# YuePanEdward/MULLS

Measured on NVIDIA H100. Metric: scan-pair registrations/sec (120k-pt 64-beam), higher is better.
Workload: dtype f32 geometry / f64 accumulation

## Files before the change

### mulls_b200/csrc/kernels_iterate.cuh

```cuda
#pragma once
#include <cooperative_groups.h>

#include "device_math.cuh"
#include "device_types.cuh"
#include "kernels_ingest.cuh"

namespace mulls {

__device__ __forceinline__ bool chunk_in_run(const DeviceArrays &A) { return blockIdx.x < (unsigned)A.ctl->n_it_chunks; }
__device__ __forceinline__ int loop_buf(const DeviceArrays &A, int buf) { return buf >= 0 ? buf : (A.ctl->it & 1); }
__device__ __forceinline__ mulls_icp_trace *trace_of(const DeviceArrays &A, uint32_t pair) {
    return (A.trace && A.ctl->trace_on) ? &A.trace[pair] : nullptr;
}

template <class Body>
__device__ __forceinline__ void for_each_live_chunk(const DeviceArrays &A, int parity, int which, Body body) {
    __shared__ uint32_t s_fetch;
    LoopCtl &ctl = *A.ctl;
    const uint32_t n = ctl.n_live[parity];
    const uint32_t *list = A.live_chunks + (size_t)parity * A.live_stride;
    for (;;) {
        __syncthreads();
        if (threadIdx.x == 0) s_fetch = atomicAdd(&ctl.work[which], 1u);
        __syncthreads();
// ... 482 lines not shown
    t[19] = (-wx * py * pz);
    t[20] = wx * py * py + wy * px * px;
    t[21] = (-wx * dx);
    t[22] = (-wy * dy);
    t[23] = (-wz * dz);
    t[24] = wy * pz * dy - wz * py * dz;
    t[25] = wz * px * dz - wx * pz * dx;
    t[26] = wx * py * dx - wy * px * dy;
}

__device__ __forceinline__ float balanced_ground_weight(const PairConst &pc, const uint32_t *n_corr) {
    if (!pc.w_balance) return 1.0f;
    const int m1 = (int)(n_corr[MULLS_GROUND] + n_corr[MULLS_ROOF]);
    const int m2 = (int)n_corr[MULLS_FACADE], m3 = (int)n_corr[MULLS_PILLAR], m4 = (int)n_corr[MULLS_BEAM];
    const float num = pc.z_xy_ratio * (float)(m2 + 2 * m3 - m4);
    const double v = (double)num / (0.0001 + 2.0 * (double)m1);
    return (float)((0.01 > v) ? 0.01 : v);
}

__device__ __forceinline__ bool too_few(const PairConst &pc, const PairState &ps, const uint32_t *n_corr, float &ratio) {
    int total = 0;
    for (int c = 0; c < kNumClasses; ++c) total += (int)n_corr[c];
    const int nec = (int)(n_corr[MULLS_PILLAR] + n_corr[MULLS_BEAM] + n_corr[MULLS_FACADE]);
    ratio = (float)(1.0 * (double)nec / (double)ps.source_feature_points_count);
    return total < 40 || nec < 20 || ratio < pc.min_ratio;
}

__device__ __forceinline__ void pair_left_running(DeviceArrays &A) {
    const int left = atomicSub(A.running, 1) - 1;
    *A.h_running = left;
    __threadfence_system();
}

__device__ __noinline__ void solve_and_advance(DeviceArrays &A, uint32_t pair, const double *S, double *sm ,
                                  int buf_written) {
    const PairConst &pc = A.pc[pair];
    PairState &ps = A.ps[pair];
    const int i = ps.iter;
    ps.iters_entered = i + 1;
    for (int c = 0; c < kNumClasses; ++c) ps.n_corr_last[c] = ps.n_corr[c];
    {
        uint64_t pts = 0;
        for (int c = 0; c < kNumClasses; ++c)
            if (pc.used[c]) pts += (uint64_t)ps.n_tgt[c];
        ps.alg_bytes += 28ull * pts;
    }
    mulls_icp_trace *tr = trace_of(A, pair);
    if (tr && i < MULLS_MAX_TRACE_ITERS) {
        tr->n_iter = i + 1;
        for (int c = 0; c < kNumClasses; ++c) tr->n_corr[i][c] = ps.n_corr[c];
        for (int k = 0; k < 36; ++k) tr->atpa[i][k] = 0.0;
        for (int k = 0; k < 6; ++k) tr->atpb[i][k] = tr->x[i][k] = 0.0;
    }
    float ratio;
    const bool few = too_few(pc, ps, ps.n_corr, ratio);
    ps.confidence = ratio;
    if (few) {
        ps.code = -2;
        ps.status = kDone;
        pair_left_running(A);
        return;
    }
    {
        const double t = 1.0 * (double)ps.thre / (double)pc.thre_rate;
        ps.thre = (t > (double)pc.thre_min) ? (float)t : pc.thre_min;
    }
    double *ATPA = sm;
    double *ATPb = sm + 36;
    double *inv = sm + 42;
    double *lu = sm + 78;
    double *Tmp = sm + 114;
    double low[21];
    for (int k = 0; k < 21; ++k) low[k] = 0.0;
    for (int k = 0; k < 6; ++k) ATPb[k] = 0.0;
    const int order[6] = {MULLS_GROUND, MULLS_FACADE, MULLS_ROOF, MULLS_PILLAR, MULLS_BEAM, MULLS_VERTEX};
    for (int o = 0; o < 6; ++o) {
        const double *s = S + order[o] * kTerms;
        for (int k = 0; k < 21; ++k) low[k] += s[k];
        for (int k = 0; k < 6; ++k) ATPb[k] += s[21 + k];
    }
    {
        int k = 0;
        for (int col = 0; col < 6; ++col)
            for (int row = col; row < 6; ++row, ++k) {
                ATPA[6 * row + col] = low[k];
                ATPA[6 * col + row] = low[k];
            }
    }
    inverse6(ATPA, inv, lu);
    double x[6];
    for (int r = 0; r < 6; ++r) {
        double s = inv[6 * r] * ATPb[0];
        for (int cc = 1; cc < 6; ++cc) s = s + inv[6 * r + cc] * ATPb[cc];
        x[r] = s;
        ps.x[r] = s;
    }
    if (tr && i < MULLS_MAX_TRACE_ITERS) {
        for (int k = 0; k < 36; ++k) tr->atpa[i][k] = ATPA[k];
        for (int k = 0; k < 6; ++k) {
            tr->atpb[i][k] = ATPb[k];
            tr->x[i][k] = x[k];
        }
    }
    {
        const float sr = (float)sin(0.5 * x[3]), sp = (float)sin(0.5 * x[4]), sy = (float)sin(0.5 * x[5]);
        const float cr = (float)cos(0.5 * x[3]), cp = (float)cos(0.5 * x[4]), cy = (float)cos(0.5 * x[5]);
        double J[3][3];
        J[0][0] = 0.5 * (double)(cr * cp * cy + sr * sp * sy);
        J[0][1] = 0.5 * (double)(-sr * sp * cy - cr * cp * sy);
        J[0][2] = 0.5 * (double)(-sr * cp * sy - cr * sp * cy);
        J[1][0] = 0.5 * (double)(-sr * sp * cy + cr * cp * sy);
        J[1][1] = 0.5 * (double)(cr * cp * cy - sr * sp * sy);
        J[1][2] = 0.5 * (double)(-cr * sp * sy + sr * cp * cy);
        J[2][0] = 0.5 * (double)(-sr * cp * sy - cr * sp * cy);
        J[2][1] = 0.5 * (double)(-cr * sp * sy - sr * cp * cy);
        J[2][2] = 0.5 * (double)(cr * cp * cy + sr * sp * sy);
        double *cof = ps.cofactor;
        for (int k = 0; k < 36; ++k) cof[k] = inv[k];
        double tmp[3][3];
        for (int r = 0; r < 3; ++r)
            for (int cc = 0; cc < 3; ++cc)
                tmp[r][cc] = J[r][0] * inv[6 * 3 + 3 + cc] + J[r][1] * inv[6 * 4 + 3 + cc] + J[r][2] * inv[6 * 5 + 3 + cc];
        for (int r = 0; r < 3; ++r)
            for (int cc = 0; cc < 3; ++cc)
                cof[6 * (3 + r) + 3 + cc] = tmp[r][0] * J[cc][0] + tmp[r][1] * J[cc][1] + tmp[r][2] * J[cc][2];
        for (int r = 0; r < 3; ++r)
            for (int cc = 0; cc < 3; ++cc)
                cof[6 * r + 3 + cc] = inv[6 * r + 3] * J[cc][0] + inv[6 * r + 4] * J[cc][1] + inv[6 * r + 5] * J[cc][2];
        for (int r = 0; r < 3; ++r)
            for (int cc = 0; cc < 3; ++cc)
                cof[6 * (3 + r) + cc] = J[r][0] * inv[6 * 3 + cc] + J[r][1] * inv[6 * 4 + cc] + J[r][2] * inv[6 * 5 + cc];
    }
    double *Tt = ps.T_inc;
    construct_trans_a(x, Tt);
    const double ts_norm = sqrt(Tt[3] * Tt[3] + Tt[7] * Tt[7] + Tt[11] * Tt[11]);
    const double rs_angle = fabs(rotation_angle(Tt));
    if (ts_norm > (double)pc.max_t || rs_angle > (double)pc.max_r) {
        ps.code = -1;
        ps.status = kDone;
        pair_left_running(A);
        return;
    }
    mat4_mul(Tt, ps.T_total, Tmp);
    for (int k = 0; k < 16; ++k) ps.T_total[k] = Tmp[k];
    if (i == pc.max_iter - 1 || (i > 2 && ts_norm < (double)pc.conv_t && rs_angle < (double)pc.conv_r)) {
        ps.status = kNeedPosterior;
        ps.final_buf = buf_written;
        pair_left_running(A);
        return;
    }
    ps.iter = i + 1;
}

__device__ __forceinline__ void accumulate_body(DeviceArrays &A, int buf, uint32_t chunk) {
    const ChunkDesc cd = A.it_chunks[chunk];
    const PairConst &pc = A.pc[cd.pair];
    PairState &ps = A.ps[cd.pair];
    if (ps.status != kRunning) return;
    const int c = (int)cd.seg;
    const int ns = ps.n_src[c];
    const uint32_t local = cd.first + threadIdx.x;
    const bool valid = (int)local < ns;
    const int lane = threadIdx.x & 31, warp = threadIdx.x >> 5;
    constexpr int kWarps = kIterBlock / 32;
    __shared__ double s_terms[27 * kIterBlock];
    __shared__ uint32_t s_off[kWarps + 1];
    __shared__ uint32_t s_base;

    if ((int)cd.first >= ns) return;
    uint32_t dst_local = 0;
    uint8_t fl = 0;
    uint32_t gi = 0;
    bool kept = false, pass = false;
    struct Column {
        double *base;
        __device__ __forceinline__ double &operator[](int k) const { return base[k * kIterBlock]; }
    } t = {s_terms + threadIdx.x};
    {
        uint32_t acc = 0;
        const uint32_t first_chunk = pc.class_chunk_begin[c];
        for (uint32_t b = first_chunk + threadIdx.x; b < chunk; b += kIterBlock) acc += A.blk_kept[b];
        for (int o = 16; o > 0; o >>= 1) acc += __shfl_xor_sync(0xffffffffu, acc, o);
        if (lane == 0) s_off[warp] = acc;
        __syncthreads();
        if (threadIdx.x == 0) {
            uint32_t tt = 0;
            for (int w = 0; w < kWarps; ++w) tt += s_off[w];
            s_base = tt;
        }
        __syncthreads();
    }
    if (valid) {
        gi = pc.src_base[c] + local;
        fl = A.flags[gi];
    }
    kept = (fl & 1) != 0, pass = (fl & 2) != 0;
    const unsigned kb = __ballot_sync(0xffffffffu, kept);
    if (lane == 0) s_off[warp] = __popc(kb);
    __syncthreads();
    if (threadIdx.x == 0) {
        uint32_t run = 0;
        for (int w = 0; w < kWarps; ++w) {
            const uint32_t tt = s_off[w];
            s_off[w] = run;
            run += tt;
        }
        s_off[kWarps] = run;
    }
    __syncthreads();
    dst_local = s_base + s_off[warp] + __popc(kb & ((1u << lane) - 1u));

    float4 p = make_float4(0, 0, 0, 0);
    int j = -1;
    float d2 = 0.0f;
    const uint32_t gd = pc.src_base[c] + dst_local;
    if (kept) {
        p = advanced_pos(ps, A.src_pos[buf][gi]);
        j = A.nn_idx[gi];
        d2 = A.nn_d2[gi];
        if (j >= 0) A.claim[pc.tgt_base[c] + j] = kClaimFree;
        A.src_pos[buf ^ 1][gd] = p;
        A.src_nrm[buf ^ 1][gd] = advanced_nrm(ps, A.src_nrm[buf][gi]);
        A.src_prevj[buf ^ 1][gd] = j;
        if (ps.iter >= kKeepFromIter - 1) A.src_cert[buf ^ 1][gd] = A.src_cert[buf][gi];
    }
    float w_store = 0.0f;
    uint32_t n_corr[kNumClasses];
#pragma unroll
    for (int k = 0; k < kNumClasses; ++k) n_corr[k] = ps.n_corr[k];
    float ratio_unused;
    const bool few = too_few(pc, ps, n_corr, ratio_unused);
    if (pass && !few) {
        const float4 q = A.tgt_pos[pc.tgt_base[c] + j];
        const float4 qn = A.tgt_nrm[pc.tgt_base[c] + j];
        const int it = ps.iter;
        const bool resid_w = pc.w_residual && it > 2;
        const bool dist_w = pc.w_dist != 0, inten_w = pc.w_intensity != 0;
        if (c == MULLS_GROUND || c == MULLS_FACADE || c == MULLS_ROOF) {
            const float wc = (c == MULLS_FACADE) ? 1.0f : balanced_ground_weight(pc, n_corr);
            terms_pt2pl(p, p.w, q, qn, wc, it, dist_w, resid_w, inten_w, pc.win_pt2pl, t, w_store);
        } else if (c == MULLS_PILLAR || c == MULLS_BEAM) {
            terms_pt2li(p, p.w, q, qn, 1.0f, it, dist_w, resid_w, inten_w, pc.win_pt2li, t, w_store);
        } else {
            terms_pt2pt(p, p.w, q, 1.0f, it, dist_w, resid_w, inten_w, pc.win_pt2pt, t);
            w_store = d2;
        }
    } else {
#pragma unroll
        for (int k = 0; k < 27; ++k) t[k] = 0.0;
    }
    if (kept) {
        A.corr_j[gd] = pass ? j : -1;
        A.corr_w[gd] = w_store;
    }
    __syncthreads();
#pragma unroll 1
    for (int k = warp; k < 27; k += kWarps) {
        const double *row = s_terms + k * kIterBlock;
        double v = ((row[lane] + row[lane + 32]) + row[lane + 64]) + row[lane + 96];
#pragma unroll
        for (int o = 16; o > 0; o >>= 1) v += __shfl_xor_sync(0xffffffffu, v, o);
        if (lane == 0) A.partials[(size_t)chunk * kTerms + k] = v;
    }
}
__global__ void __launch_bounds__(kIterBlock, 8) k_accumulate(DeviceArrays A, int buf) {
    buf = loop_buf(A, buf);
    if (blockIdx.x == 0 && threadIdx.x == 0) A.ctl->work[0] = 0u;
    for_each_live_chunk(A, buf, 2, [&](uint32_t chunk) { accumulate_body(A, buf, chunk); });
}

__device__ __forceinline__ void publish_live_chunks(const DeviceArrays &A, uint32_t pair, int next_parity) {
    __shared__ uint32_t s_base;
    __syncthreads();
    const PairConst &pc = A.pc[pair];
    const PairState &ps = A.ps[pair];
    if (ps.status != kRunning) return;
    uint32_t count[kNumClasses], total = 0;
#pragma unroll
    for (int c = 0; c < kNumClasses; ++c) {
        count[c] = (uint32_t)((ps.n_src[c] + kIterBlock - 1) / kIterBlock);
        total += count[c];
    }
    if (threadIdx.x == 0) s_base = atomicAdd(&A.ctl->n_live[next_parity], total);
    __syncthreads();
    uint32_t base = s_base;
#pragma unroll
    for (int c = 0; c < kNumClasses; ++c) {
        append_live_chunks(A, next_parity, pc.class_chunk_begin[c], count[c], base);
        base += count[c];
    }
}

__device__ __forceinline__ void solve_body(DeviceArrays &A, int buf, uint32_t pair) {
    const PairConst &pc = A.pc[pair];
    PairState &ps = A.ps[pair];
    if (ps.status != kRunning) return;
    const int lane = threadIdx.x & 31, warp = threadIdx.x >> 5, n_warps = blockDim.x >> 5;
    __shared__ double s_S[kNumClasses][kTerms];
    __shared__ double s_scratch[160];
    __shared__ int s_newn[kNumClasses];
    __shared__ uint32_t s_ncorr[kNumClasses];
    for (int cc = warp; cc < kNumClasses; cc += n_warps) {
        const uint32_t b0 = pc.class_chunk_begin[cc];
        const uint32_t live = (uint32_t)((ps.n_src[cc] + kIterBlock - 1) / kIterBlock);
        const uint32_t b1 = min(pc.class_chunk_begin[cc + 1], b0 + live);
        double a0 = 0.0, a1 = 0.0, a2 = 0.0, a3 = 0.0;
        if (lane < 27) {
            uint32_t b = b0;
            for (; b + 4 <= b1; b += 4) {
                a0 += A.partials[(size_t)(b + 0) * kTerms + lane];
                a1 += A.partials[(size_t)(b + 1) * kTerms + lane];
                a2 += A.partials[(size_t)(b + 2) * kTerms + lane];
                a3 += A.partials[(size_t)(b + 3) * kTerms + lane];
            }
            for (; b < b1; ++b) a0 += A.partials[(size_t)b * kTerms + lane];
        }
        if (lane < kTerms) s_S[cc][lane] = (lane < 27) ? ((a0 + a1) + (a2 + a3)) : 0.0;
        uint32_t acc = 0;
        for (uint32_t b = b0 + lane; b < b1; b += 32) acc += A.blk_kept[b];
        for (int o = 16; o > 0; o >>= 1) acc += __shfl_xor_sync(0xffffffffu, acc, o);
        if (lane == 0) {
            s_newn[cc] = (int)acc;
            s_ncorr[cc] = ps.n_corr[cc];
        }
    }
    __syncthreads();
    if (threadIdx.x == 0) {
        uint64_t srcpts = 0;
        for (int cc = 0; cc < kNumClasses; ++cc)
            if (pc.used[cc]) srcpts += (uint64_t)ps.n_src_g[cc];
        ps.alg_bytes += 28ull * srcpts;
        if (pc.sharded) {
            for (int cc = 0; cc < kNumClasses; ++cc) {
                ps.n_src[cc] = s_newn[cc];
                for (int k = 0; k < kTerms; ++k) A.xch_f64[cc * kTerms + k] = (k < 27) ? s_S[cc][k] : 0.0;
            }
        } else {
        mulls_icp_trace *tr = trace_of(A, pair);
        for (int cc = 0; cc < kNumClasses; ++cc) {
            ps.n_src[cc] = s_newn[cc];
            ps.n_src_g[cc] = s_newn[cc];
            ps.n_corr[cc] = s_ncorr[cc];
            if (tr && ps.iter < MULLS_MAX_TRACE_ITERS) tr->n_src[ps.iter][cc] = (uint32_t)ps.n_src[cc];
        }
        solve_and_advance(A, pair, &s_S[0][0], s_scratch, buf ^ 1);
        for (int cc = 0; cc < kNumClasses; ++cc) ps.n_corr[cc] = 0;
        }
    }
    if (!pc.sharded) publish_live_chunks(A, pair, buf ^ 1);
}
constexpr int kSolveThreads = kNumClasses * 32;
__global__ void __launch_bounds__(kSolveThreads) k_solve(DeviceArrays A, int buf, unsigned long long loop_handle) {
    LoopCtl &ctl = *A.ctl;
    if (blockIdx.x >= (unsigned)ctl.n_pairs) return;
    solve_body(A, loop_buf(A, buf), blockIdx.x);
    if (loop_handle == 0ull) return;
    __syncthreads();
    if (threadIdx.x == 0) {
        __threadfence();
        if (atomicAdd(&ctl.solved, 1u) == (unsigned)ctl.n_pairs - 1u) {
            ctl.solved = 0;
            const int it = ctl.it + 1;
            ctl.it = it;
            __threadfence();
            const bool again = *(volatile int *)A.running > 0 && it < ctl.max_iter;
            cudaGraphSetConditional((cudaGraphConditionalHandle)loop_handle, again ? 1u : 0u);
        }
    }
}

__global__ void __launch_bounds__(kIterBlock, 4) k_icp_loop(DeviceArrays A) {
    namespace cg = cooperative_groups;
    cg::grid_group grid = cg::this_grid();
    LoopCtl &ctl = *A.ctl;
    __shared__ uint8_t s_need[kIterBlock];
    __shared__ float4 s_carry[kIterBlock];
    __shared__ uint32_t s_n_need;
    const int n_pairs = ctl.n_pairs, max_iter = ctl.max_iter;
    for (int it = 0; it < max_iter; ++it) {
        const int buf = it & 1;
        const uint32_t *list = A.live_chunks + (size_t)buf * A.live_stride;
        const uint32_t n_live = ctl.n_live[buf];
        if (blockIdx.x == 0 && threadIdx.x == 0) ctl.n_live[buf ^ 1] = 0u;
        const int mode = search_mode_of(it);
        for (uint32_t w = blockIdx.x; w < n_live; w += gridDim.x) {
            const uint32_t chunk = list[w];
            if (mode == 2) search_keep_chunk(A, buf, chunk, s_need, s_carry, &s_n_need);
            else if (mode == 1) search_quarter<WalkBounds>(A, buf, chunk, threadIdx.x >> 5, true);
            else search_quarter<NoBounds>(A, buf, chunk, threadIdx.x >> 5, false);
            __syncthreads();
        }
        grid.sync();
        for (uint32_t w = blockIdx.x; w < n_live; w += gridDim.x) {
            resolve_body(A, buf, list[w]);
            __syncthreads();
        }
        grid.sync();
        for (uint32_t w = blockIdx.x; w < n_live; w += gridDim.x) {
            accumulate_body(A, buf, list[w]);
            __syncthreads();
        }
        grid.sync();
        for (int pair = blockIdx.x; pair < n_pairs; pair += gridDim.x) {
            solve_body(A, buf, (uint32_t)pair);
            __syncthreads();
        }
        grid.sync();
        if (*(volatile int *)A.running <= 0) break;
    }
}

__global__ void k_shard_pack_setup(DeviceArrays A, int phase) {
    PairState &ps = A.ps[0];
    if (phase == 0) {
        for (int d = 0; d < 3; ++d) {
            A.xch_i32[d] = ps.bb_src[d];
            A.xch_i32[3 + d] = ~ps.bb_src[3 + d];
        }
    } else if (phase == 1) {
        for (int d = 0; d < 3; ++d) {
            ps.bb_src[d] = A.xch_i32[d];
            ps.bb_src[3 + d] = ~A.xch_i32[3 + d];
        }
    } else if (phase == 2) {
        for (int c = 0; c < kNumClasses; ++c) A.xch_i32[c] = ps.n_src[c];
    } else {
        const PairConst &pc = A.pc[0];
        int cnt = 0;
        for (int c = 0; c < kNumClasses; ++c) ps.n_src_g[c] = A.xch_i32[c];
        if (pc.used[MULLS_PILLAR]) cnt += ps.n_src_g[MULLS_PILLAR];
        if (pc.used[MULLS_FACADE]) cnt += ps.n_src_g[MULLS_FACADE];
        if (pc.used[MULLS_BEAM]) cnt += ps.n_src_g[MULLS_BEAM];
        ps.source_feature_points_count = cnt;
    }
}
__global__ void __launch_bounds__(kIterBlock) k_shard_counts(DeviceArrays A, int phase) {
    const PairConst &pc = A.pc[0];
    PairState &ps = A.ps[0];
    if (ps.status != kRunning) {
        if (phase == 0 && threadIdx.x < 2 * kNumClasses) A.xch_i32[threadIdx.x] = 0;
        return;
    }
    if (phase == 0) {
        __shared__ uint32_t s_w[kIterBlock / 32];
        for (int cc = 0; cc < kNumClasses; ++cc) {
            const uint32_t b0 = pc.class_chunk_begin[cc];
            const uint32_t live = (uint32_t)((ps.n_src[cc] + kIterBlock - 1) / kIterBlock);
            const uint32_t b1 = min(pc.class_chunk_begin[cc + 1], b0 + live);
            uint32_t acc = 0;
            for (uint32_t b = b0 + threadIdx.x; b < b1; b += kIterBlock) acc += A.blk_kept[b];
            for (int o = 16; o > 0; o >>= 1) acc += __shfl_xor_sync(0xffffffffu, acc, o);
            __syncthreads();
            if ((threadIdx.x & 31) == 0) s_w[threadIdx.x >> 5] = acc;
            __syncthreads();
            if (threadIdx.x == 0) {
                uint32_t tot = 0;
                for (int w = 0; w < kIterBlock / 32; ++w) tot += s_w[w];
                A.xch_i32[kNumClasses + cc] = (int)tot;
                A.xch_i32[cc] = (int)ps.n_corr[cc];
            }
        }
    } else if (threadIdx.x == 0) {
        for (int cc = 0; cc < kNumClasses; ++cc) {
            ps.n_corr[cc] = (uint32_t)A.xch_i32[cc];
            ps.n_src_g_next[cc] = A.xch_i32[kNumClasses + cc];
        }
    }
}
__global__ void k_shard_solve(DeviceArrays A, int buf, int it_flag) {
    PairState &ps = A.ps[0];
    __shared__ double s_scratch[160];
    if (threadIdx.x == 0) {
        if (ps.status != kRunning) {
            A.h_running_iter[it_flag] = *A.running;
            __threadfence_system();
        } else {
            mulls_icp_trace *tr = trace_of(A, 0);
            for (int cc = 0; cc < kNumClasses; ++cc) {
                ps.n_src_g[cc] = ps.n_src_g_next[cc];
                if (tr && ps.iter < MULLS_MAX_TRACE_ITERS) tr->n_src[ps.iter][cc] = (uint32_t)ps.n_src_g[cc];
            }
            solve_and_advance(A, 0, A.xch_f64, s_scratch, buf ^ 1);
            for (int cc = 0; cc < kNumClasses; ++cc) ps.n_corr[cc] = 0;
            A.h_running_iter[it_flag] = *A.running;
            __threadfence_system();
        }
    }
    publish_live_chunks(A, 0, buf ^ 1);
}
__global__ void k_shard_post(DeviceArrays A, int phase) {
    const PairConst &pc = A.pc[0];
    PairState &ps = A.ps[0];
    if (threadIdx.x != 0) return;
    if (phase == 0) {
        double VTPV = 0.0, nob = 0.0;
        if (ps.status == kNeedPosterior) {
            const int order[6] = {MULLS_GROUND, MULLS_FACADE, MULLS_ROOF, MULLS_PILLAR, MULLS_BEAM, MULLS_VERTEX};
            for (int o = 0; o < 6; ++o) {
                const uint32_t b0 = pc.class_chunk_begin[order[o]];
                const uint32_t live = (uint32_t)((ps.n_src[order[o]] + kIterBlock - 1) / kIterBlock);
                const uint32_t b1 = min(pc.class_chunk_begin[order[o] + 1], b0 + live);
                for (uint32_t b = b0; b < b1; ++b) {
                    VTPV += A.post_partials[2 * (size_t)b];
                    nob += A.post_partials[2 * (size_t)b + 1];
                }
            }
        }
        A.xch_f64[0] = VTPV;
        A.xch_f64[1] = nob;
    } else if (ps.status == kNeedPosterior) {
        const double sigma2 = A.xch_f64[0] / (double)((int)A.xch_f64[1] - 6);
        ps.sigma2 = sigma2;
        ps.code = (sqrt(sigma2) < pc.sigma_thre) ? 1 : -3;
        double inv[36], lu[36];
        inverse6(ps.cofactor, inv, lu);
        for (int k = 0; k < 36; ++k) ps.info[k] = (1.0 / sigma2) * inv[k];
        ps.status = kDone;
    }
}

__global__ void __launch_bounds__(kIterBlock) k_posterior(DeviceArrays A) {
    if (!chunk_in_run(A)) return;
    const ChunkDesc cd = A.it_chunks[blockIdx.x];
    const PairConst &pc = A.pc[cd.pair];
    PairState &ps = A.ps[cd.pair];
    if (ps.status != kNeedPosterior) return;
    const int c = (int)cd.seg;
    const int buf = ps.final_buf;
    if ((int)cd.first >= ps.n_src[c]) return;
    const uint32_t local = cd.first + threadIdx.x;
    const bool valid = (int)local < ps.n_src[c];
    double vtpv = 0.0;
    int nobs = 0;
    if (valid) {
        const uint32_t gi = pc.src_base[c] + local;
        const int j = A.corr_j[gi];
        if (j >= 0) {
            const float4 p = A.src_pos[buf][gi];
            const float4 q = A.tgt_pos[pc.tgt_base[c] + j];
            const float4 qn = A.tgt_nrm[pc.tgt_base[c] + j];
            const float w = A.corr_w[gi];
            const double *x = ps.x;
            const float px = p.x, py = p.y, pz = p.z, qx = q.x, qy = q.y, qz = q.z;
            if (c == MULLS_GROUND || c == MULLS_FACADE || c == MULLS_ROOF) {
                const float ntx = qn.x, nty = qn.y, ntz = qn.z;
                const float a = ntz * py - nty * pz;
                const float b = ntx * pz - ntz * px;
                const float cc = nty * px - ntx * py;
                const float d = ntx * qx + nty * qy + ntz * qz - ntx * px - nty * py - ntz * pz;
                const float residual = (float)((double)ntx * x[0] + (double)nty * x[1] + (double)ntz * x[2] +
                                               (double)a * x[3] + (double)b * x[4] + (double)cc * x[5] - (double)d);
                vtpv = (double)(w * residual * residual);
// ... 148 lines not shown
```

### mulls_b200/csrc/mulls_b200.cu

```cuda
#include <algorithm>
#include <atomic>
#include <memory>
#include <cmath>
#include <cstdio>
#include <chrono>
#include <cstring>
#include <string>
#include <vector>

#include <cub/device/device_radix_sort.cuh>
#include <cub/device/device_scan.cuh>
#include <cub/device/device_select.cuh>

#include <dlfcn.h>
#include <mutex>

#include "device_types.cuh"
#include "host_pack.h"
#include "scan_io.h"
#include "kernels_ingest.cuh"
#include "kernels_iterate.cuh"
#include "kernels_pca.cuh"
#include "kernels_map.cuh"
#include "kernels_classify.cuh"
// ... 620 lines not shown
                for (size_t f = 0; f < v.n; f += kJobPts) {
                    jobs.push_back(PackJob{v.aos48, pos, nrm, f, std::min(kJobPts, v.n - f), fmt, &pending[p]});
                    ++n_jobs;
                }
                slot += packed_slots(v.n, fmt);
            }
            pending[p].store(n_jobs, std::memory_order_relaxed);
        }
        slot_begin[n_pairs] = slot;
        if (slot > ctx->h_stage_slots || slot > 3 * ctx->cap_in) {
            ctx->err = "internal: packed staging capacity";
            return MULLS_E_CAPACITY;
        }
        pool.submit(jobs);
        cudaError_t ce = cudaMemcpyAsync(ctx->A.pc, ctx->h_pc.data(), n_pairs * sizeof(PairConst), cudaMemcpyHostToDevice, ctx->stream);
        if (ce == cudaSuccess && !ctx->h_in_chunks.empty())
            ce = cudaMemcpyAsync(ctx->A.in_chunks, ctx->h_in_chunks.data(), ctx->h_in_chunks.size() * sizeof(ChunkDesc),
                                 cudaMemcpyHostToDevice, ctx->stream);
        if (ce == cudaSuccess && !ctx->h_it_chunks.empty())
            ce = cudaMemcpyAsync(ctx->A.it_chunks, ctx->h_it_chunks.data(), ctx->h_it_chunks.size() * sizeof(ChunkDesc),
                                 cudaMemcpyHostToDevice, ctx->stream);
        tables_sent = true;
        if (ce == cudaSuccess && cudaEventRecord(ctx->ev_h2d0, ctx->stream) == cudaSuccess) ctx->h2d_timed = true;
        const double t_pack0 = wall_ms();
        for (size_t p = 0; p < n_pairs; ++p) {
            pool.help_until_done(pending[p]);
            if (p + 1 == n_pairs) ctx->up_ms_pack = (float)(wall_ms() - t_pack0);
            const size_t b = slot_begin[p], e = slot_begin[p + 1];
            if (e > b && ce == cudaSuccess)
                ce = cudaMemcpyAsync((void *)(ctx->A.in_aos + b), ctx->h_stage + b, (e - b) * sizeof(float4), cudaMemcpyHostToDevice,
                                     ctx->stream);
        }
        CK(ce);
    } else {
    if (cudaEventRecord(ctx->ev_h2d0, ctx->stream) == cudaSuccess) ctx->h2d_timed = true;
    for (size_t p = 0; p < n_pairs; ++p) {
        PairConst &pc = ctx->h_pc[p];
        for (int s = 0; s < kNumSegs; ++s) {
            const mulls_cloud_view &v = (s < kNumClasses) ? tgt[p * kNumClasses + s] : src[p * kNumClasses + (s - kNumClasses)];
            pc.in_ptr[s] = ctx->A.in_aos + 3 * (size_t)pc.in_off[s];
            pc.in_fmt[s] = kFmtRows48;
            if (v.n == 0) continue;
            if (tgt_on_device && s < kNumClasses) {
                pc.in_ptr[s] = (const float4 *)v.aos48;
                continue;
            }
            CK(cudaMemcpyAsync((void *)(ctx->A.in_aos + 3 * (size_t)pc.in_off[s]), v.aos48, v.n * 48, cudaMemcpyHostToDevice,
                               ctx->stream));
        }
    }
    }
    if (!tables_sent) {
        CK(cudaMemcpyAsync(ctx->A.pc, ctx->h_pc.data(), n_pairs * sizeof(PairConst), cudaMemcpyHostToDevice, ctx->stream));
        if (!ctx->h_in_chunks.empty())
            CK(cudaMemcpyAsync(ctx->A.in_chunks, ctx->h_in_chunks.data(), ctx->h_in_chunks.size() * sizeof(ChunkDesc),
                               cudaMemcpyHostToDevice, ctx->stream));
        if (!ctx->h_it_chunks.empty())
            CK(cudaMemcpyAsync(ctx->A.it_chunks, ctx->h_it_chunks.data(), ctx->h_it_chunks.size() * sizeof(ChunkDesc),
                               cudaMemcpyHostToDevice, ctx->stream));
    }
    if (resident) CK(cudaStreamSynchronize(ctx->stream));
    ctx->n_pairs = n_pairs;
    ctx->n_in = in_off;
    ctx->n_src_total = s_off;
    ctx->n_tgt_total = t_off;
    ctx->max_iter_max = max_iter_max;
    ctx->any_keep_less = any_keep_less;
    ctx->any_normal_shooting = any_shoot;
    ctx->any_undistort = any_undistort;
    ctx->uploaded = true;
    ctx->up_ms_host = (float)(wall_ms() - t_up0);
    return MULLS_OK;
}

static int exchange(mulls_ctx *ctx, mulls_allreduce_fn hook, void *user, void *buf, size_t count, int dtype, int op) {
    if (hook(user, buf, count, dtype, op, (void *)ctx->stream) == 0) return MULLS_OK;
    ctx->err = "all-reduce callback failed";
    return MULLS_E_COMM;
}

static int launch_ingest(mulls_ctx *ctx, DeviceArrays &A, bool trace, uint64_t &launches, mulls_allreduce_fn hook = nullptr,
                         void *user = nullptr, bool finite_only = false) {
    cudaStream_t st = ctx->stream;
    const int np = (int)ctx->n_pairs;
    const uint32_t n_in = (uint32_t)ctx->n_in;
    if (trace) CK(cudaMemsetAsync(ctx->d_trace, 0, np * sizeof(mulls_icp_trace), st));
    CK(cudaMemsetAsync(A.claim, 0x7f, std::max<size_t>(ctx->n_tgt_total, 1) * sizeof(unsigned), st));
    k_state_init<<<(unsigned)ceil_div(np, 128), 128, 0, st>>>(A, np);
    ++launches;
    const unsigned n_inc = (unsigned)ctx->h_in_chunks.size();
    if (n_inc) {
        if (ctx->any_undistort) k_ingest_bbox<true><<<n_inc, kIngestBlock, 0, st>>>(A);
        else if (finite_only) k_ingest_bbox<false, true><<<n_inc, kIngestBlock, 0, st>>>(A);
        else k_ingest_bbox<false><<<n_inc, kIngestBlock, 0, st>>>(A);
        ++launches;
    }
    if (hook) {
        k_shard_pack_setup<<<1, 1, 0, st>>>(A, 0);
        if (const int rc = exchange(ctx, hook, user, A.xch_i32, 6, 1, 1); rc != MULLS_OK) return rc;
        k_shard_pack_setup<<<1, 1, 0, st>>>(A, 1);
        launches += 2;
    }
    k_pair_setup<<<(unsigned)ceil_div(np, 128), 128, 0, st>>>(A, np);
    ++launches;
    if (n_inc) {
        if (ctx->any_undistort) k_make_keys<true><<<n_inc, kIngestBlock, 0, st>>>(A);
        else if (finite_only) k_make_keys<false, true><<<n_inc, kIngestBlock, 0, st>>>(A);
        else k_make_keys<false><<<n_inc, kIngestBlock, 0, st>>>(A);
        ++launches;
        if (ctx->any_keep_less) {
            const unsigned pb = (unsigned)ceil_div(np, 64);
            k_keepless_plan<<<pb, 64, 0, st>>>(A, np);
            for (int pass = 0; pass < 8; ++pass) {
                k_keepless_hist<<<n_inc, kIngestBlock, 0, st>>>(A, pass);
                k_keepless_step<<<pb, 64, 0, st>>>(A, np, pass);
            }
            k_keepless_mark<<<n_inc, kIngestBlock, 0, st>>>(A);
            launches += 18;
        }
        int seg_bits = 1;
        while ((1ull << seg_bits) <= (uint64_t)np * kNumSegs) ++seg_bits;
        size_t bytes = ctx->cub_temp_bytes;
        CK(cub::DeviceRadixSort::SortPairs(ctx->cub_temp, bytes, A.keys_a, A.keys_b, A.vals_a, A.vals_b, (int)n_in, 0,
                                           36 + seg_bits, st));
    }
    k_seg_offsets<<<1, 256, 0, st>>>(A, np);
    ++launches;
    if (hook) {
        k_shard_pack_setup<<<1, 1, 0, st>>>(A, 2);
        if (const int rc = exchange(ctx, hook, user, A.xch_i32, kNumClasses, 1, 0); rc != MULLS_OK) return rc;
        k_shard_pack_setup<<<1, 1, 0, st>>>(A, 3);
        launches += 2;
    }
    if (n_in) {
        const unsigned nb = (unsigned)ceil_div(n_in, 256);
        if (ctx->any_undistort) k_gather<true><<<nb, 256, 0, st>>>(A, A.keys_b, A.vals_b, n_in);
        else k_gather<false><<<nb, 256, 0, st>>>(A, A.keys_b, A.vals_b, n_in);
        k_hash_layout<<<1, 32, 0, st>>>(A, np);
        k_hash_clear<<<1184, 256, 0, st>>>(A);
        k_hash_build<<<nb, 256, 0, st>>>(A, A.keys_b, n_in);
        launches += 4;
    } else {
        k_hash_layout<<<1, 32, 0, st>>>(A, np);
        ++launches;
    }
    return MULLS_OK;
}

static unsigned chunk_bucket(const mulls_ctx *ctx) {
    unsigned b = 1;
    while (b < (unsigned)ctx->h_it_chunks.size()) b <<= 1;
    return b;
}
static unsigned resident_grid(const mulls_ctx *ctx, int blocks_per_sm) {
    return std::min((unsigned)(ctx->num_sms * blocks_per_sm), chunk_bucket(ctx));
}
constexpr int kShootBlocksPerSm = 8, kAccumulateBlocksPerSm = 8;
constexpr int kPollPause = 64;

static int enqueue_iteration(mulls_ctx *ctx, int it, mulls_allreduce_fn hook, void *user, unsigned long long handle,
                             uint64_t &launches) {
    cudaStream_t st = ctx->stream;
    const DeviceArrays &A = ctx->A;
    const bool recording = it < 0;
    const int buf = recording ? -1 : it & 1;
    if (hook)
        CK(cudaMemsetAsync(A.claim, 0x7f, std::max<size_t>(ctx->n_tgt_total, 1) * sizeof(unsigned), st));
    if (!recording) CK(cudaEventRecord(ctx->ev_search[2 * it], st));
    const unsigned search_grid = resident_grid(ctx, kSearchBlocksPerSm);
    const int mode = recording ? -1 : search_mode_of(it);
    if (mode < 0 || mode == 0) k_search<0><<<search_grid, kIterBlock, 0, st>>>(A, buf, it);
    if (mode < 0 || mode == 1) k_search<1><<<search_grid, kIterBlock, 0, st>>>(A, buf, it);
    if (mode < 0 || mode == 2) k_search<2><<<search_grid, kIterBlock, 0, st>>>(A, buf, it);
    launches += recording ? 3 : 1;
    if (ctx->any_normal_shooting) {
        k_search_shoot<<<resident_grid(ctx, kShootBlocksPerSm), kIterBlock, 0, st>>>(A, buf);
        ++launches;
    }
    if (!recording) CK(cudaEventRecord(ctx->ev_search[2 * it + 1], st));
    if (hook) {
        if (const int rc = exchange(ctx, hook, user, A.claim, ctx->n_tgt_total, 1, 1); rc != MULLS_OK) return rc;
    }
    k_resolve<<<resident_grid(ctx, kResolveBlocksPerSm), kIterBlock, 0, st>>>(A, buf);
    if (hook) {
        k_shard_counts<<<1, kIterBlock, 0, st>>>(A, 0);
        if (const int rc = exchange(ctx, hook, user, A.xch_i32, 2 * kNumClasses, 1, 0); rc != MULLS_OK) return rc;
        k_shard_counts<<<1, kIterBlock, 0, st>>>(A, 1);
        launches += 2;
    }
    k_accumulate<<<resident_grid(ctx, kAccumulateBlocksPerSm), kIterBlock, 0, st>>>(A, buf);
    k_solve<<<recording ? (unsigned)std::max<size_t>(ctx->max_pairs, 1) : (unsigned)ctx->n_pairs, kSolveThreads, 0, st>>>(A, buf, handle);
    launches += 3;
    if (hook) {
        if (const int rc = exchange(ctx, hook, user, A.xch_f64, kNumClasses * kTerms, 0, 0); rc != MULLS_OK) return rc;
        k_shard_solve<<<1, 32, 0, st>>>(A, buf, it);
        ++launches;
    }
    return MULLS_OK;
}

static int enqueue_tail(mulls_ctx *ctx, bool recording, mulls_allreduce_fn hook, void *user, uint64_t &launches) {
    cudaStream_t st = ctx->stream;
    const DeviceArrays &A = ctx->A;
    const unsigned pairs = recording ? (unsigned)std::max<size_t>(ctx->max_pairs, 1) : (unsigned)ctx->n_pairs;
    const int np = recording ? -1 : (int)ctx->n_pairs;
    k_posterior<<<recording ? std::min((unsigned)std::max<size_t>(ctx->cap_it_chunks, 1), chunk_bucket(ctx))
                            : (unsigned)ctx->h_it_chunks.size(), kIterBlock, 0, st>>>(A);
    if (hook) {
        k_shard_post<<<1, 32, 0, st>>>(A, 0);
        if (const int rc = exchange(ctx, hook, user, A.xch_f64, 2, 0, 0); rc != MULLS_OK) return rc;
        k_shard_post<<<1, 32, 0, st>>>(A, 1);
    } else {
        k_finalize<<<(unsigned)ceil_div(pairs, 64), 64, 0, st>>>(A, np);
    }
    if (!recording) CK(cudaEventRecord(ctx->ev_iter, st));
    k_collect<<<(unsigned)ceil_div(pairs, 128), 128, 0, st>>>(A, np, ctx->d_results);
    launches += hook ? 4 : 3;
    return MULLS_OK;
}

static int build_iteration_graph(mulls_ctx *ctx) {
    const int key[2] = {(int)chunk_bucket(ctx), ctx->any_normal_shooting ? 1 : 0};
    if (ctx->graph_exec && std::memcmp(key, ctx->graph_key, sizeof(key)) == 0) return MULLS_OK;
    drop_iteration_graph(ctx);
    cudaStream_t st = ctx->stream;
    const int rc = [&]() -> int {
        CK(cudaGraphCreate(&ctx->graph, 0));
        cudaGraphConditionalHandle handle;
        CK(cudaGraphConditionalHandleCreate(&handle, ctx->graph, 1, cudaGraphCondAssignDefault));
        cudaGraphNodeParams wp = {cudaGraphNodeTypeConditional};
        wp.conditional.handle = handle;
        wp.conditional.type = cudaGraphCondTypeWhile;
        wp.conditional.size = 1;
        cudaGraphNode_t while_node;
        CK(cudaGraphAddNode(&while_node, ctx->graph, nullptr, 0, &wp));
        uint64_t body = 0, tail = 0;
        CK(cudaStreamBeginCaptureToGraph(st, wp.conditional.phGraph_out[0], nullptr, nullptr, 0, cudaStreamCaptureModeThreadLocal));
        int rc = enqueue_iteration(ctx, -1, nullptr, nullptr, (unsigned long long)handle, body);
        CK(cudaStreamEndCapture(st, nullptr));
        if (rc != MULLS_OK) return rc;
        CK(cudaStreamBeginCaptureToGraph(st, ctx->graph, &while_node, nullptr, 1, cudaStreamCaptureModeThreadLocal));
        rc = enqueue_tail(ctx, true, nullptr, nullptr, tail);
        CK(cudaStreamEndCapture(st, nullptr));
        if (rc != MULLS_OK) return rc;
        CK(cudaGraphInstantiate(&ctx->graph_exec, ctx->graph, 0));
        ctx->graph_body_launches = body, ctx->graph_tail_launches = tail;
        return MULLS_OK;
    }();
    if (rc != MULLS_OK) return drop_iteration_graph(ctx), rc;
    std::memcpy(ctx->graph_key, key, sizeof(key));
    return MULLS_OK;
}

static int grow_hash_pool(mulls_ctx *ctx) {
    const uint32_t need = ctx->h_flags[2];
    DeviceArrays &A = ctx->A;
    if (need <= A.hash_pool_entries || need == 0xffffffffu) {
        ctx->err = "hash pool exhausted (the target clouds need " + std::to_string(need) + " grid entries)";
        return MULLS_E_CAPACITY;
    }
    HashEntry *fresh = nullptr;
    if (cudaMalloc(&fresh, (size_t)need * sizeof(HashEntry)) != cudaSuccess) {
        cudaGetLastError();
        ctx->err = "hash pool exhausted, and no device memory to grow it to " + std::to_string(need) + " entries";
        return MULLS_E_CAPACITY;
    }
    std::replace(ctx->allocs.begin(), ctx->allocs.end(), (void *)A.hash, (void *)fresh);
    CK(cudaFree(A.hash));
    A.hash = fresh;
    A.hash_pool_entries = need;
    drop_iteration_graph(ctx);
    return MULLS_OK;
}

static int drain_on_error(mulls_ctx *ctx, int rc) {
    if (rc != MULLS_OK && ctx && ctx->stream) cudaStreamSynchronize(ctx->stream);
    return rc;
}

static int run_finish(mulls_ctx *ctx, mulls_icp_result *out);
static int run_impl(mulls_ctx *ctx, mulls_icp_result *out, mulls_icp_trace *trace, mulls_allreduce_fn hook, void *user,
                    bool finish_now = true) {
    return drain_on_error(ctx, [&]() -> int {
        if (!ctx || !ctx->uploaded) return MULLS_E_ARG;
        ctx->pend.active = false;
        CK(cudaSetDevice(ctx->device));
        cudaStream_t st = ctx->stream;
        DeviceArrays A = ctx->A;
        const int np = (int)ctx->n_pairs;
        uint64_t launches = 0;
        CK(cudaEventRecord(ctx->ev_begin, st));
        if (const int rc = launch_ingest(ctx, A, trace != nullptr, launches, hook, user); rc != MULLS_OK) return rc;
        const unsigned n_itc = (unsigned)ctx->h_it_chunks.size();
        {
            LoopCtl &c = *ctx->h_ctl;
            c = LoopCtl();
            c.n_it_chunks = (int)n_itc, c.n_pairs = np, c.trace_on = trace ? 1 : 0, c.max_iter = ctx->max_iter_max;
            CK(cudaMemcpyAsync(A.ctl, ctx->h_ctl, sizeof(LoopCtl), cudaMemcpyHostToDevice, st));
            k_live_init<<<(unsigned)ceil_div(n_itc, 256), 256, 0, st>>>(A);
            ++launches;
        }
        bool looped = false;
        if (!hook && ctx->use_graph && !ctx->any_normal_shooting) {
            if (ctx->loop_kernel_blocks == 0) {
                int per_sm = 0, coop = 0;
                cudaDeviceGetAttribute(&coop, cudaDevAttrCooperativeLaunch, ctx->device);
                if (coop && cudaOccupancyMaxActiveBlocksPerMultiprocessor(&per_sm, k_icp_loop, kIterBlock, 0) == cudaSuccess && per_sm > 0)
                    ctx->loop_kernel_blocks = per_sm * ctx->num_sms;
                else
                    ctx->loop_kernel_blocks = -1, cudaGetLastError();
            }
            looped = ctx->loop_kernel_blocks > 0 && n_itc <= (unsigned)ctx->loop_kernel_blocks && np <= ctx->loop_kernel_blocks;
        }
        const bool graphed = !hook && ctx->use_graph && !looped;
        if (const int rc = graphed ? build_iteration_graph(ctx) : MULLS_OK; rc != MULLS_OK) return rc;
        CK(cudaEventRecord(ctx->ev_ingest, st));
        int n_search_ev = 0;
        if (graphed) {
            CK(cudaGraphLaunch(ctx->graph_exec, st));
            CK(cudaMemcpyAsync(ctx->h_ctl, A.ctl, sizeof(LoopCtl), cudaMemcpyDeviceToHost, st));
            CK(cudaEventRecord(ctx->ev_iter, st));
        } else {
            if (looped) {
                DeviceArrays Aarg = A;
                void *args[] = {&Aarg};
                const unsigned grid = std::max(1u, std::min((unsigned)ctx->loop_kernel_blocks, std::max(n_itc, (unsigned)np)));
                CK(cudaLaunchCooperativeKernel((const void *)k_icp_loop, dim3(grid), dim3(kIterBlock), args, 0, st));
                ++launches;
            } else {
                for (int it = 0; it < ctx->max_iter_max; ++it) {
                    if (it >= 2) {
                        while (cudaEventQuery(ctx->ev_done[it - 2]) == cudaErrorNotReady)
                            for (int k = 0; k < kPollPause; ++k) _mm_pause();
                        if (hook ? ((volatile int *)ctx->h_running)[1 + (it - 2)] <= 0 : *(volatile int *)ctx->h_running <= 0) break;
                    }
                    if (const int rc = enqueue_iteration(ctx, it, hook, user, 0ull, launches); rc != MULLS_OK) return rc;
                    CK(cudaEventRecord(ctx->ev_done[it], st));
                    n_search_ev = it + 1;
                }
            }
            if (const int rc = enqueue_tail(ctx, false, hook, user, launches); rc != MULLS_OK) return rc;
        }
        CK(cudaMemcpyAsync(ctx->h_results, ctx->d_results, np * (sizeof(mulls_icp_result) + sizeof(uint64_t)), cudaMemcpyDeviceToHost, st));
// ... 1719 lines not shown
```

Before: 6386.

## Accumulate ICP terms one chunk per warp with register reduction

Restructures the standalone accumulate kernel so each warp claims a whole chunk from the work queue and loops over its 32-lane slots, keeping the 27 f64 terms in registers and reducing them with warp shuffles. This removes the large shared-memory staging buffer and the block-wide syncs and prefix scans. The grid shrinks to match, and blocks per SM drops to 4 to allow the extra registers. The cooperative path keeps a block-level variant through a shared helper. The risks are higher register pressure and lower occupancy from 27 f64 accumulators per thread.

```diff
diff --git a/mulls_b200/csrc/kernels_iterate.cuh b/mulls_b200/csrc/kernels_iterate.cuh
--- a/mulls_b200/csrc/kernels_iterate.cuh
+++ b/mulls_b200/csrc/kernels_iterate.cuh
@@ -658,7 +658,118 @@
     ps.iter = i + 1;
 }
 
-__device__ __forceinline__ void accumulate_body(DeviceArrays &A, int buf, uint32_t chunk) {
+template <class Emit>
+__device__ __forceinline__ void accumulate_source(DeviceArrays &A, const PairConst &pc, const PairState &ps, int c,
+                                                  int buf, int it, uint32_t gi, uint32_t gd, uint32_t fl, bool few,
+                                                  const uint32_t *n_corr, Emit emit) {
+    const bool kept = (fl & 1) != 0, pass = (fl & 2) != 0;
+    float4 p = make_float4(0, 0, 0, 0);
+    int j = -1;
+    float d2 = 0.0f;
+    if (kept) {
+        p = advanced_pos(ps, A.src_pos[buf][gi]);
+        j = A.nn_idx[gi];
+        d2 = A.nn_d2[gi];
+        if (j >= 0) A.claim[pc.tgt_base[c] + j] = kClaimFree;
+        A.src_pos[buf ^ 1][gd] = p;
+        A.src_nrm[buf ^ 1][gd] = advanced_nrm(ps, A.src_nrm[buf][gi]);
+        A.src_prevj[buf ^ 1][gd] = j;
+        if (it >= kKeepFromIter - 1) A.src_cert[buf ^ 1][gd] = A.src_cert[buf][gi];
+    }
+    float w_store = 0.0f;
+    double t[27];
+    if (pass && !few) {
+        const float4 q = A.tgt_pos[pc.tgt_base[c] + j];
+        const float4 qn = A.tgt_nrm[pc.tgt_base[c] + j];
+        const bool resid_w = pc.w_residual && it > 2;
+        const bool dist_w = pc.w_dist != 0, inten_w = pc.w_intensity != 0;
+        if (c == MULLS_GROUND || c == MULLS_FACADE || c == MULLS_ROOF) {
+            const float wc = (c == MULLS_FACADE) ? 1.0f : balanced_ground_weight(pc, n_corr);
+            terms_pt2pl(p, p.w, q, qn, wc, it, dist_w, resid_w, inten_w, pc.win_pt2pl, t, w_store);
+            emit(t);
+        } else if (c == MULLS_PILLAR || c == MULLS_BEAM) {
+            terms_pt2li(p, p.w, q, qn, 1.0f, it, dist_w, resid_w, inten_w, pc.win_pt2li, t, w_store);
+            emit(t);
+        } else {
+            terms_pt2pt(p, p.w, q, 1.0f, it, dist_w, resid_w, inten_w, pc.win_pt2pt, t);
+            w_store = d2;
+            emit(t);
+        }
+    } else {
+        constexpr double kZeros[27] = {};
+        emit(kZeros);
+    }
+    if (kept) {
+        A.corr_j[gd] = pass ? j : -1;
+        A.corr_w[gd] = w_store;
+    }
+}
+
+constexpr int kAccumulateBlocksPerSm = 4;
+__device__ __forceinline__ void accumulate_chunk_warp(DeviceArrays &A, int buf, uint32_t chunk) {
+    const ChunkDesc cd = A.it_chunks[chunk];
+    const PairConst &pc = A.pc[cd.pair];
+    PairState &ps = A.ps[cd.pair];
+    if (ps.status != kRunning) return;
+    const int c = (int)cd.seg;
+    const int ns = ps.n_src[c];
+    if ((int)cd.first >= ns) return;
+    const int lane = threadIdx.x & 31;
+    constexpr int kSlots = kIterBlock / 32;
+    const uint32_t first = pc.src_base[c] + cd.first;
+    uint32_t fl = 0;
+#pragma unroll
+    for (int s = 0; s < kSlots; ++s)
+        if ((int)cd.first + 32 * s + lane < ns) fl |= (uint32_t)A.flags[first + 32 * s + lane] << (8 * s);
+    uint32_t dst = 0;
+#pragma unroll 4
+    for (uint32_t b = pc.class_chunk_begin[c] + lane; b < chunk; b += 32) dst += A.blk_kept[b];
+    for (int o = 16; o > 0; o >>= 1) dst += __shfl_xor_sync(0xffffffffu, dst, o);
+    uint32_t n_corr[kNumClasses];
+#pragma unroll
+    for (int k = 0; k < kNumClasses; ++k) n_corr[k] = ps.n_corr[k];
+    float ratio_unused;
+    const bool few = too_few(pc, ps, n_corr, ratio_unused);
+    const int it = ps.iter;
+    double acc[27];
+#pragma unroll
+    for (int k = 0; k < 27; ++k) acc[k] = -0.0;
+#pragma unroll 1
+    for (int s = 0; s < kSlots; ++s, fl >>= 8) {
+        const unsigned kb = __ballot_sync(0xffffffffu, (fl & 1) != 0);
+        const uint32_t gd = pc.src_base[c] + dst + __popc(kb & ((1u << lane) - 1u));
+        dst += __popc(kb);
+        accumulate_source(A, pc, ps, c, buf, it, first + 32 * s + lane, gd, fl, few, n_corr, [&acc](const double *t) {
+#pragma unroll
+            for (int k = 0; k < 27; ++k) acc[k] += t[k];
+        });
+    }
+    double mine = 0.0;
+#pragma unroll
+    for (int k = 0; k < 27; ++k) {
+        double v = acc[k];
+#pragma unroll
+        for (int o = 16; o > 0; o >>= 1) v += __shfl_xor_sync(0xffffffffu, v, o);
+        if (lane == k) mine = v;
+    }
+    if (lane < 27) A.partials[(size_t)chunk * kTerms + lane] = mine;
+}
+__global__ void __launch_bounds__(kIterBlock, kAccumulateBlocksPerSm) k_accumulate(DeviceArrays A, int buf) {
+    buf = loop_buf(A, buf);
+    LoopCtl &ctl = *A.ctl;
+    if (blockIdx.x == 0 && threadIdx.x == 0) ctl.work[0] = 0u;
+    const uint32_t n = ctl.n_live[buf];
+    const uint32_t *list = A.live_chunks + (size_t)buf * A.live_stride;
+    for (;;) {
+        uint32_t w = 0;
+        if ((threadIdx.x & 31) == 0) w = atomicAdd(&ctl.work[2], 1u);
+        w = __shfl_sync(0xffffffffu, w, 0);
+        if (w >= n) break;
+        accumulate_chunk_warp(A, buf, list[w]);
+    }
+}
+
+__device__ __forceinline__ void accumulate_chunk_block(DeviceArrays &A, int buf, uint32_t chunk) {
     const ChunkDesc cd = A.it_chunks[chunk];
     const PairConst &pc = A.pc[cd.pair];
     PairState &ps = A.ps[cd.pair];
@@ -674,14 +785,8 @@
     __shared__ uint32_t s_base;
 
     if ((int)cd.first >= ns) return;
-    uint32_t dst_local = 0;
     uint8_t fl = 0;
     uint32_t gi = 0;
-    bool kept = false, pass = false;
-    struct Column {
-        double *base;
-        __device__ __forceinline__ double &operator[](int k) const { return base[k * kIterBlock]; }
-    } t = {s_terms + threadIdx.x};
     {
         uint32_t acc = 0;
         const uint32_t first_chunk = pc.class_chunk_begin[c];
@@ -700,8 +805,7 @@
         gi = pc.src_base[c] + local;
         fl = A.flags[gi];
     }
-    kept = (fl & 1) != 0, pass = (fl & 2) != 0;
-    const unsigned kb = __ballot_sync(0xffffffffu, kept);
+    const unsigned kb = __ballot_sync(0xffffffffu, (fl & 1) != 0);
     if (lane == 0) s_off[warp] = __popc(kb);
     __syncthreads();
     if (threadIdx.x == 0) {
@@ -714,51 +818,16 @@
         s_off[kWarps] = run;
     }
     __syncthreads();
-    dst_local = s_base + s_off[warp] + __popc(kb & ((1u << lane) - 1u));
-
-    float4 p = make_float4(0, 0, 0, 0);
-    int j = -1;
-    float d2 = 0.0f;
-    const uint32_t gd = pc.src_base[c] + dst_local;
-    if (kept) {
-        p = advanced_pos(ps, A.src_pos[buf][gi]);
-        j = A.nn_idx[gi];
-        d2 = A.nn_d2[gi];
-        if (j >= 0) A.claim[pc.tgt_base[c] + j] = kClaimFree;
-        A.src_pos[buf ^ 1][gd] = p;
-        A.src_nrm[buf ^ 1][gd] = advanced_nrm(ps, A.src_nrm[buf][gi]);
-        A.src_prevj[buf ^ 1][gd] = j;
-        if (ps.iter >= kKeepFromIter - 1) A.src_cert[buf ^ 1][gd] = A.src_cert[buf][gi];
-    }
-    float w_store = 0.0f;
+    const uint32_t gd = pc.src_base[c] + s_base + s_off[warp] + __popc(kb & ((1u << lane) - 1u));
     uint32_t n_corr[kNumClasses];
 #pragma unroll
     for (int k = 0; k < kNumClasses; ++k) n_corr[k] = ps.n_corr[k];
     float ratio_unused;
     const bool few = too_few(pc, ps, n_corr, ratio_unused);
-    if (pass && !few) {
-        const float4 q = A.tgt_pos[pc.tgt_base[c] + j];
-        const float4 qn = A.tgt_nrm[pc.tgt_base[c] + j];
-        const int it = ps.iter;
-        const bool resid_w = pc.w_residual && it > 2;
-        const bool dist_w = pc.w_dist != 0, inten_w = pc.w_intensity != 0;
-        if (c == MULLS_GROUND || c == MULLS_FACADE || c == MULLS_ROOF) {
-            const float wc = (c == MULLS_FACADE) ? 1.0f : balanced_ground_weight(pc, n_corr);
-            terms_pt2pl(p, p.w, q, qn, wc, it, dist_w, resid_w, inten_w, pc.win_pt2pl, t, w_store);
-        } else if (c == MULLS_PILLAR || c == MULLS_BEAM) {
-            terms_pt2li(p, p.w, q, qn, 1.0f, it, dist_w, resid_w, inten_w, pc.win_pt2li, t, w_store);
-        } else {
-            terms_pt2pt(p, p.w, q, 1.0f, it, dist_w, resid_w, inten_w, pc.win_pt2pt, t);
-            w_store = d2;
-        }
-    } else {
-#pragma unroll
-        for (int k = 0; k < 27; ++k) t[k] = 0.0;
-    }
-    if (kept) {
-        A.corr_j[gd] = pass ? j : -1;
-        A.corr_w[gd] = w_store;
-    }
+    accumulate_source(A, pc, ps, c, buf, ps.iter, gi, gd, fl, few, n_corr, [](const double *t) {
+#pragma unroll
+        for (int k = 0; k < 27; ++k) s_terms[k * kIterBlock + threadIdx.x] = t[k];
+    });
     __syncthreads();
 #pragma unroll 1
     for (int k = warp; k < 27; k += kWarps) {
@@ -768,11 +837,6 @@
         for (int o = 16; o > 0; o >>= 1) v += __shfl_xor_sync(0xffffffffu, v, o);
         if (lane == 0) A.partials[(size_t)chunk * kTerms + k] = v;
     }
-}
-__global__ void __launch_bounds__(kIterBlock, 8) k_accumulate(DeviceArrays A, int buf) {
-    buf = loop_buf(A, buf);
-    if (blockIdx.x == 0 && threadIdx.x == 0) A.ctl->work[0] = 0u;
-    for_each_live_chunk(A, buf, 2, [&](uint32_t chunk) { accumulate_body(A, buf, chunk); });
 }
 
 __device__ __forceinline__ void publish_live_chunks(const DeviceArrays &A, uint32_t pair, int next_parity) {
@@ -903,7 +967,7 @@
         }
         grid.sync();
         for (uint32_t w = blockIdx.x; w < n_live; w += gridDim.x) {
-            accumulate_body(A, buf, list[w]);
+            accumulate_chunk_block(A, buf, list[w]);
             __syncthreads();
         }
         grid.sync();
diff --git a/mulls_b200/csrc/mulls_b200.cu b/mulls_b200/csrc/mulls_b200.cu
--- a/mulls_b200/csrc/mulls_b200.cu
+++ b/mulls_b200/csrc/mulls_b200.cu
@@ -796,10 +796,10 @@
     while (b < (unsigned)ctx->h_it_chunks.size()) b <<= 1;
     return b;
 }
-static unsigned resident_grid(const mulls_ctx *ctx, int blocks_per_sm) {
-    return std::min((unsigned)(ctx->num_sms * blocks_per_sm), chunk_bucket(ctx));
-}
-constexpr int kShootBlocksPerSm = 8, kAccumulateBlocksPerSm = 8;
+static unsigned resident_grid(const mulls_ctx *ctx, int blocks_per_sm, unsigned chunks_per_block = 1) {
+    return std::min((unsigned)(ctx->num_sms * blocks_per_sm), (chunk_bucket(ctx) + chunks_per_block - 1) / chunks_per_block);
+}
+constexpr int kShootBlocksPerSm = 8;
 constexpr int kPollPause = 64;
 
 static int enqueue_iteration(mulls_ctx *ctx, int it, mulls_allreduce_fn hook, void *user, unsigned long long handle,
@@ -832,7 +832,7 @@
         k_shard_counts<<<1, kIterBlock, 0, st>>>(A, 1);
         launches += 2;
     }
-    k_accumulate<<<resident_grid(ctx, kAccumulateBlocksPerSm), kIterBlock, 0, st>>>(A, buf);
+    k_accumulate<<<resident_grid(ctx, kAccumulateBlocksPerSm, kIterBlock / 32), kIterBlock, 0, st>>>(A, buf);
     k_solve<<<recording ? (unsigned)std::max<size_t>(ctx->max_pairs, 1) : (unsigned)ctx->n_pairs, kSolveThreads, 0, st>>>(A, buf, handle);
     launches += 3;
     if (hook) {
```

Result: faster. 6609, median of 6 (+3.5%).
